# joncampbell123/composite-video-simulator

Hardware: AMD Instinct MI355X
Metric: frames/sec (output frames = fields; 720x486 NTSC, preset '-vhs'; steady-state pipelined throughput, 4 steps in flight) (higher is better)
Workload: dtype f64; 1 GPU; 720x486 30fps 10s colour-bars clip, preset '-vhs': 300 frames -> 600 fields per GPU per step, frame-round-robin over 1 GPU(s); steps_in_flight=4, mode=exact (bit-identical to the reference: fp64, no FMA contraction)

## Files before the change

composite-video-simulator_amd/csrc/ntsc_decode_fast.hip:

```cpp
#include "ntsc_pack.hpp"
#include "ntsc_rowend_plan.hpp"

#pragma clang fp contract(off)

namespace ntscsim {
namespace fastdec {

typedef uint32_t v4u __attribute__((ext_vector_type(4)));
#ifdef NTSC_PLAIN_OUT_STORES
#define NTSC_OUT_STORE(p, v) (*(p) = (v))
#else
#define NTSC_OUT_STORE(p, v) __builtin_nontemporal_store((v), (p))
#endif
typedef __attribute__((address_space(1))) v4u *g_v4u_ptr;
typedef __attribute__((address_space(1))) const v4u *g_cv4u_ptr;
DEV v4u to_v4u(const uint4 &a) { return v4u{a.x, a.y, a.z, a.w}; }
typedef __attribute__((address_space(1))) uint32_t *g_u32_ptr;
typedef __attribute__((address_space(1))) const uint32_t *g_cu32_ptr;

#ifdef NTSC_NO_STEP_SCHED_BARRIER
#define NTSC_STEP_SCHED_BARRIER() ((void)0)
#else
#define NTSC_STEP_SCHED_BARRIER() __builtin_amdgcn_sched_barrier(0)
#endif
// ... 182 lines not shown
        if (pick_next) { e1 = D.w4; e2 = D.w2; o1 = D.w5; o2 = D.w3; }
        else           { e1 = D.w5; e2 = D.w3; o1 = D.w4; o2 = D.w2; }
        y0 = D.y0; y1 = D.y1; y2 = D.y2; y3 = D.y3; y4 = D.y4;
        ieP = D.ieP; qeP = D.qeP; ieN = D.ieN; qeN = D.qeN;
    }
    DEV void to(DemodR &D, bool pick_next) const
    {
        D.c2 = c1; D.c1 = pA - c1; D.c0 = pB - D.c1; D.csum = D.c0 + D.c1 + D.c2;
        D.w0 = 0; D.w1 = 0;
        if (pick_next) { D.w4 = e1; D.w2 = e2; D.w5 = o1; D.w3 = o2; }
        else           { D.w5 = e1; D.w3 = e2; D.w4 = o1; D.w2 = o2; }
        D.y0 = y0; D.y1 = y1; D.y2 = y2; D.y3 = y3; D.y4 = y4;
        D.ieP = ieP; D.qeP = qeP; D.ieN = ieN; D.qeN = qeN;
    }
    template <bool PICK, bool NEG, bool LUMA, bool BK = false, bool MASK = false, bool ANY = false>
    DEV void push(int ct, bool hi, int dm, int &Yo, int &Io, int &Qo, unsigned bmul = 0, unsigned bshift = 0,
                  bool odd = false, int mo = 0)
    {
        const int p = ct + c1;
        const int yb = sdiv4s(p + pB);
        int ch = ct - yb;
        if (BK) ch = scale_back50(ch, bmul, bshift);
        c1 = ct; pB = pA; pA = p;
        if (LUMA) { Yo = y0; y0 = y1; y1 = y2; y2 = y3; y3 = y4; y4 = yb; }
        if (PICK) {
            int a, b;
            if (ANY) {
                const int aL = odd ? o2 : e2, aH = odd ? o1 : e1;
                const int bL = odd ? e1 : o2, bH = odd ? ch : o1;
                a = hi ? aH : aL; b = hi ? bH : bL;
                const int sg = NEG ? ~mo : mo;
                a = (a ^ sg) - sg; b = (b ^ sg) - sg;
            } else {
                a = hi ? e1 : e2; b = hi ? o1 : o2;
                if (NEG) { a = -a; b = -b; }
            }
            e2 = e1; e1 = ch;
            if (MASK) { a &= dm; b &= dm; }
            ieN = a; qeN = b;
            Io = (ieP + ieN) >> 1;
            Qo = (qeP + qeN) >> 1;
        } else {
            o2 = o1; o1 = ch;
            Io = ieN; Qo = qeN;
            ieP = ieN; qeP = qeN;
        }
    }
};

template <bool VHS, class RT>
struct State {
    DemodR D1, D2;
    int l0, l1, l2, lsum;
    Casc3<RT> vl, vcU, vcV, sh, oU, oV;
    PoleHp<RT> vpre;
    int Yprev, Uraw, Vraw;
    RT Uf2[2];
    LaneRand32 rng;
    int nU, nV;
};

template <class RT, bool WR = false, bool BK = false, bool SV = false, bool XA = false, bool FO = false>
struct Const {
    static constexpr bool fullout = FO;
    static constexpr int SH = FO ? 3 : 0;
    RT a_oi, a_oq;
    uint32_t *xs;
    static constexpr bool wraps = WR;
    static constexpr bool back = BK;
    static constexpr bool svideo = SV;
    static constexpr bool anyxi = XA;
    bool odd;
    int mo;
    int ms[4];
    unsigned bmul, bshift;
    int wrapoff;
    int wrapA, wrapS;
    unsigned xi;
    bool hi;
    int W, xe, lane;
    int d, SKT, LOFF;
// ... 48 lines not shown
    g = g < 0 ? 0 : (g > 255 ? 255 : g);
    b = b < 0 ? 0 : (b > 255 ? 255 : b);
    return (((uint32_t)r << 16) | (uint32_t)b) | ((uint32_t)g << 8);
#else
    const uint32_t r = cvt_sat_u32((y + (RT(0.956) * fU)) + (RT(0.621) * fV));
    const uint32_t g = cvt_sat_u32((y + (RT(-0.272) * fU)) + (RT(-0.647) * fV));
    const uint32_t b = cvt_sat_u32((y + (RT(-1.106) * fU)) + (RT(1.703) * fV));
    return pack_bgra(r, g, b);
#endif
}

struct Steady {
    DemodS D1, D2;
    int lc1, lpA, lpB;
    uint32_t *rb;
    bool rb0;
    int yd[4];
    int ud[2];
};

template <int DPH, int J, class RT, class CT>
DEV int vcr_step(const DevParams &P, State<true, RT> &S, Steady &T, const CT &C,
                 int pc, int pl, int &Yv, int &Uv, int &Vv)
{
    constexpr bool pick1 = ((DPH + J) & 1) != 0;
    constexpr bool neg1 = ((DPH + J) & 3) == 3;
    int Yd, U, V;
    T.D1.template push<pick1, neg1, false, CT::back, false, CT::anyxi>(pc, C.hi, -1, Yd, U, V, C.bmul, C.bshift, C.odd, C.mo);
    U += S.nU; V += S.nV;
    S.nU = noise_next(S.nU, S.rng.template draw<2 * J>(T.rb, T.rb0), P.m_cnoise, P.cnoise_k);
    S.nV = noise_next(S.nV, S.rng.template draw<2 * J + 1>(T.rb, T.rb0), P.m_cnoise, P.cnoise_k);
    const RT u = (RT)U, v = (RT)V;
    const RT Ud = rtrunc<RT>((u * C.cosv) - (v * C.sinv));
    const RT Vd = rtrunc<RT>((u * C.sinv) + (v * C.cosv));
    const int fU = (int)S.vcU.push(Ud, C.a_vc);
    const int fV = (int)S.vcV.push(Vd, C.a_vc);
    const int lp = pl + T.lc1;
    const int yb = sdiv4s(lp + T.lpB);
    T.lc1 = pl; T.lpB = T.lpA; T.lpA = lp;
    RT m2;
    RT s = S.vl.push((RT)yb, C.a_vl, m2);
    s += S.vpre.hp(s, m2, C.a_vl) * RT(1.6);
    const RT s0 = rtrunc<RT>(s);
    const RT ts = S.sh.push(s0, C.a_sh);
    const int Y = (int)(s0 + ((s0 - ts) * C.sharp2));
    U = ((wave_up(fU) & C.bA) + fU + C.bC) >> C.bC;
    V = ((wave_up(fV) & C.bA) + fV + C.bC) >> C.bC;
    Yv = Y; Uv = U; Vv = V;
    constexpr int J2 = (J + CT::SH) & 3;
    if constexpr (CT::anyxi) {
        const int chroma = (J2 & 1) ? (C.odd ? U : V) : (C.odd ? V : U);
        const int mm = C.ms[J2];
        return Y + ((chroma ^ mm) - mm);
    }
    const int chroma = (J2 & 1) ? V : U;
    const int mm = (J2 & 2) ? C.mNL : C.mL;
    return Y + ((chroma ^ mm) - mm);
}

template <bool VHS, int DPH, int J, class RT, class CT>
DEV uint32_t step(const DevParams &P, State<VHS, RT> &S, Steady &T, const CT &C, int pc, int pl)
{
    int Y, U, V;
    constexpr bool pick3 = ((J + 1 + CT::SH) & 1) != 0;
    constexpr bool neg3 = ((J + 1 + CT::SH) & 3) == 3;
    if constexpr (!VHS) {
        T.D1.template push<pick3, neg3, true, CT::back, true, CT::anyxi>(pc, C.hi, C.dm, Y, U, V, C.bmul, C.bshift, C.odd, C.mo);
    } else {
        int Yv, Uv, Vv;
        const int c2 = vcr_step<DPH, J, RT, CT>(P, S, T, C, pc, pl, Yv, Uv, Vv);
        if constexpr (CT::svideo) {
            Y = Yv; U = Uv & C.dm; V = Vv & C.dm;
        } else {
            T.D2.template push<pick3, neg3, true, false, true, CT::anyxi>(c2, C.hi, C.dm, Y, U, V, 0, 0, C.odd, C.mo);
        }
    }
    if constexpr (CT::fullout) {
        const int fUn = (int)S.oU.push((RT)U, C.a_oi);
        const RT fVd = rtrunc<RT>(S.oV.push((RT)V, C.a_oq));
        const int Yo = T.yd[J];
        T.yd[J] = Y;
        const RT fUd = (RT)T.ud[J & 1];
        T.ud[J & 1] = fUn;
        return yiq_to_bgra<RT>(Yo, fUd, fVd);
    } else {
// ... 115 lines not shown
    if (in3) {
        fUd = rtrunc<RT>(S.oU.push((RT)U, C.a_tv));
        fVd = rtrunc<RT>(S.oV.push((RT)V, C.a_tv));
    }
    const int xo = x3 - 1;
    const int Yo = S.Yprev;
    const int Ur = S.Uraw, Vr = S.Vraw;
    S.Yprev = Y; S.Uraw = U; S.Vraw = V;
    if (xo < 0) return false;
    if (xo >= W - 1) { fUd = (RT)Ur; fVd = (RT)Vr; }
    px = yiq_to_bgra<RT>(Yo, fUd, fVd);
    xo_out = xo;
    return true;
}

template <bool VHS, int DPH, class RT, class CT>
DEV int steady_run(const DevParams &P, State<VHS, RT> &S, Steady &T, const CT &C, uint32_t *ring,
                   uint32_t *ostage, const unsigned long long *orow, uint32_t *drow, bool is_out, int t, int t_end,
                   int (&pc)[4], int (&pl)[4], int &sbase)
{
    const int SKT = C.SKT, LOFF = C.LOFF, lane = C.lane;
    constexpr int PD = 4;
    constexpr bool PFTOP = !VHS;
    int pend_x = -1;
#ifdef NTSC_FAST_LANE_STORE
#define NTSC_FAST_FLUSH()                                                                         \
    if (pend_x >= 0) {                                                                            \
        if (is_out) {                                                                             \
            const uint4 *sp = reinterpret_cast<const uint4 *>(&ostage[lane * 20]);                \
            g_v4u_ptr dp = (g_v4u_ptr)(drow + pend_x);                                            \
            const uint4 a = sp[0], b = sp[1], c4 = sp[2], d4 = sp[3];                             \
// ... 21 lines not shown
#endif
#ifndef NTSC_FAST_NO_ENTRY_WAIT
    __builtin_amdgcn_s_waitcnt(0x0F70);
#endif
    for (; t + 4 <= t_end; t += 4) {
        if constexpr (FLUSH_TOP) { NTSC_FAST_FLUSH() }
        uint32_t o[4];
        int nc[4] = {0, 0, 0, 0}, nl[4] = {0, 0, 0, 0};
        if (PFTOP) {
#pragma unroll
            for (int j = 0; j < 4; j++) { nc[j] = cs_load(C, t + 4 + j); nl[j] = VHS ? cs_load<NTSC_COMP_LOAD2_AUX>(C, t + 4 + j - LOFF) : 0; }
        }
        T.rb = ring + sbase * 64 + lane;
        T.rb0 = sbase == 0;
        sbase = (sbase + 8) & 31;
#define NTSC_FAST_STEP(J)                                                                         \
        o[J] = step<VHS, DPH, J, RT, CT>(P, S, T, C, pc[J % PD], pl[J % PD]);                     \
        if (!PFTOP) {                                                                             \
            pc[J % PD] = cs_load(C, t + PD + J);                                                  \
            if (VHS) pl[J % PD] = cs_load<NTSC_COMP_LOAD2_AUX>(C, t + PD + J - LOFF);                                  \
        }                                                                                         \
        NTSC_STEP_SCHED_BARRIER();
        NTSC_FAST_STEP(0)
        NTSC_FAST_STEP(1)
        NTSC_FAST_STEP(2)
        NTSC_FAST_STEP(3)
#undef NTSC_FAST_STEP
        if constexpr (PFTOP) {
#pragma unroll
            for (int j = 0; j < 4; j++) { pc[j] = nc[j]; pl[j] = nl[j]; }
        }
        const int xo0 = t - SKT;
        const int sub = (xo0 >> 2) & 3;
        *reinterpret_cast<uint4 *>(&ostage[lane * 20 + sub * 4]) = make_uint4(o[0], o[1], o[2], o[3]);
        if (sub == 3) pend_x = xo0 - 12;
// ... 31 lines not shown
    for (int j = 0; j < PD; j++) { pc[j] = cs_load(C, t + j); pl[j] = VHS ? cs_load<NTSC_COMP_LOAD2_AUX>(C, t + j - LOFF) : 0; }
    t = steady_run<VHS, DPH, RT, CT>(P, S, T, C, ring, ostage, orow, drow, is_out, t, t_end, pc, pl, sbase);
    T.D1.to(S.D1, VHS ? (DPH & 1) != 0 : pick3_next);
    T.D2.to(S.D2, pick3_next);
    if constexpr (CT::fullout) {
#pragma unroll
        for (int q = 0; q < 4; q++) C.xs[q * 64] = (uint32_t)T.yd[q];
        S.Uf2[0] = (RT)T.ud[0]; S.Uf2[1] = (RT)T.ud[1];
    }
    S.Uraw = 0; S.Vraw = 0;
    S.l2 = T.lc1; S.l1 = T.lpA - T.lc1; S.l0 = T.lpB - S.l1; S.lsum = S.l0 + S.l1 + S.l2;
    if (VHS) S.rng.pos = sbase;
    return t;
}

template <int DPH, int J, bool END, class RT, class CT>
DEV uint32_t group_step(const DevParams &P, State<true, RT> &S, Steady &T, const CT &C, const rowend::Pos &q,
                        int t, int pc, int pl)
{
    const int W = C.W;
    constexpr bool pick1 = ((DPH + J) & 1) != 0, neg1 = ((DPH + J) & 3) == 3;
    constexpr bool pick3 = ((J + 1) & 1) != 0, neg3 = ((J + 1) & 3) == 3;
    int Yd, U = 0, V = 0;
    int fU = 0, fV = 0;
    if (!END || q.sep1) {
        if constexpr (END) {
            const int x1 = t - 7;
            const int mg = pick1 ? ((x1 + 2 - W + (C.mL & 2)) >> 31) : -1;
            T.D1.template push<pick1, neg1, false, CT::back, true, false>(pc, C.hi, mg, Yd, U, V, C.bmul, C.bshift);
            if (x1 >= C.xe) { U = 0; V = 0; }
        } else {
            T.D1.template push<pick1, neg1, false, CT::back, false, false>(pc, C.hi, -1, Yd, U, V, C.bmul, C.bshift);
        }
    }
    if (q.in1) {
        U += S.nU; V += S.nV;
        S.nU = noise_next(S.nU, S.rng.template draw<2 * J>(T.rb, T.rb0), P.m_cnoise, P.cnoise_k);
        S.nV = noise_next(S.nV, S.rng.template draw<2 * J + 1>(T.rb, T.rb0), P.m_cnoise, P.cnoise_k);
        const RT u = (RT)U, v = (RT)V;
        const RT Ud = rtrunc<RT>((u * C.cosv) - (v * C.sinv));
        const RT Vd = rtrunc<RT>((u * C.sinv) + (v * C.cosv));
        fU = (int)S.vcU.push(Ud, C.a_vc);
        fV = (int)S.vcV.push(Vd, C.a_vc);
        if (END && q.tail_wr) {
            const int x1 = t - 7;
            C.tailU[(size_t)(x1 & 15) * C.rstride] = (int)Ud;
            C.tailU[(size_t)(16 + (x1 & 15)) * C.rstride] = (int)Vd;
        }
    }
    int yb;
    {
        const int lp = pl + T.lc1;
        yb = sdiv4s(lp + T.lpB);
        T.lc1 = pl; T.lpB = T.lpA; T.lpA = lp;
    }
    int c2 = 0;
    if (q.in2) {
        if (END && q.tail_rd) {
            const int x2 = t - 7 - C.d;
            fU = C.tailU[(size_t)(x2 & 15) * C.rstride];
            fV = C.tailU[(size_t)(16 + (x2 & 15)) * C.rstride];
        }
        RT m2;
        RT s = S.vl.push((RT)yb, C.a_vl, m2);
        s += S.vpre.hp(s, m2, C.a_vl) * RT(1.6);
        const RT s0 = rtrunc<RT>(s);
// ... 18 lines not shown
    }
    uint32_t px = 0;
    if (q.tv) {
        RT fUd = 0, fVd = 0;
        const int Yo = S.Yprev;
        if (q.in3) {
            fUd = rtrunc<RT>(S.oU.push((RT)U3, C.a_tv));
            fVd = rtrunc<RT>(S.oV.push((RT)V3, C.a_tv));
            S.Yprev = Y3;
        }
        if (q.out) px = yiq_to_bgra<RT>(Yo, fUd, fVd);
    }
    return px;
}

template <int DPH, bool END, class RT, class CT>
DEV void group_run(const DevParams &P, State<true, RT> &S, Steady &T, const CT &C, const rowend::Plan &RP,
                   uint32_t *ring, uint32_t *ostage, uint32_t *drow, bool is_out, int t0, int t_stop,
                   int (&pc)[4], int (&pl)[4], int &sbase)
{
    const int lane = C.lane, W = C.W;
    for (; t0 < t_stop; t0 += 4) {
        T.rb = ring + sbase * 64 + lane;
        T.rb0 = sbase == 0;
        sbase = (sbase + 8) & 31;
        uint32_t o[4] = {0u, 0u, 0u, 0u};
        bool burst = false, rest = false;
#define NTSC_GROUP_STEP(J)                                                                        \
        {                                                                                         \
            const int tj = t0 + J;           \
            const rowend::Pos q = rowend::position(RP, tj);                                       \
            o[J] = group_step<DPH, J, END, RT, CT>(P, S, T, C, q, tj, pc[J], pl[J]);              \
            burst = burst || q.burst; rest = rest || q.rest;                                      \
            const int tn = tj + 4;           \
            const rowend::Pos qn = rowend::position(RP, tn);                                      \
            pc[J] = qn.load_c ? cs_load(C, tn) : 0;                                               \
            pl[J] = qn.load_l ? cs_load<NTSC_COMP_LOAD2_AUX>(C, tn - RP.LOFF) : 0;                \
            NTSC_STEP_SCHED_BARRIER();                                                            \
        }
        NTSC_GROUP_STEP(0)
        NTSC_GROUP_STEP(1)
        NTSC_GROUP_STEP(2)
        NTSC_GROUP_STEP(3)
#undef NTSC_GROUP_STEP
        if constexpr (END) {
            const int xo0 = t0 - RP.SKT;
            const int sub = (xo0 >> 2) & 3;
            *reinterpret_cast<uint4 *>(&ostage[lane * 20 + sub * 4]) = make_uint4(o[0], o[1], o[2], o[3]);
            const int xb = xo0 & ~15;
            if (burst) {
                if (is_out) {
                    const uint4 *sp = reinterpret_cast<const uint4 *>(&ostage[lane * 20]);
                    g_v4u_ptr dp = (g_v4u_ptr)(drow + xb);
                    const uint4 a = sp[0], b = sp[1], c4 = sp[2], d4 = sp[3];
                    dp[0] = to_v4u(a); dp[1] = to_v4u(b); dp[2] = to_v4u(c4); dp[3] = to_v4u(d4);
                }
            } else if (rest && is_out) {
                for (int x = xb; x < W; x++) ((g_u32_ptr)drow)[x] = ostage[lane * 20 + (x - xb)];
            }
        }
    }
}


template <int DPH, class RT, class CT>
DEV void grouped_row(const DevParams &P, State<true, RT> &S, const CT &C, const rowend::Plan &RP, uint32_t *ring,
                     uint32_t *ostage, const unsigned long long *orow, uint32_t *drow, bool is_out)
{
    Steady T;
    T.D1.init(); T.D2.init();
    T.lc1 = T.lpA = T.lpB = 0;
    int sbase = rowend::group_slot(S.rng.pos, RP.g0);
    int pc[4], pl[4];
#pragma unroll
    for (int j = 0; j < 4; j++) {
        pc[j] = rowend::position(RP, RP.g0 + j).load_c ? cs_load(C, RP.g0 + j) : 0;
        pl[j] = 0;
    }
    group_run<DPH, false, RT, CT>(P, S, T, C, RP, ring, ostage, drow, is_out, RP.g0, RP.st0, pc, pl, sbase);
    const int t = steady_run<true, DPH, RT, CT>(P, S, T, C, ring, ostage, orow, drow, is_out, RP.st0, RP.t_end, pc, pl, sbase);
#pragma unroll
    for (int j = 0; j < 4; j++) pc[j] = rowend::position(RP, t + j).load_c ? pc[j] : 0;
    group_run<DPH, true, RT, CT>(P, S, T, C, RP, ring, ostage, drow, is_out, t, RP.glast + 4, pc, pl, sbase);
}

}

#ifndef NTSC_FAST_WAVES
#define NTSC_FAST_WAVES 2
#endif
#ifndef NTSC_FAST_WAVES_F32
#define NTSC_FAST_WAVES_F32 2
#endif
template <class RT> struct FastWaves { static constexpr int n = NTSC_FAST_WAVES; };
template <> struct FastWaves<float> { static constexpr int n = NTSC_FAST_WAVES_F32; };
template <bool VHS, class RT, bool WR, bool BK, bool SV = false, bool XA = false, bool FO = false>
DEV void decode_fast_body(const DevParams &P, const GeomDev &G, const FieldDev *__restrict__ fields,
                          const int *__restrict__ comp, const uint32_t *__restrict__ rs_chroma,
                          const int *__restrict__ n0_u, const int *__restrict__ n0_v,
                          const int *__restrict__ hs_shift, const int *__restrict__ pn_noise,
                          const int *__restrict__ dropout, int *__restrict__ tails)
{
    using namespace fastdec;
    __shared__ uint32_t ring[33 * 64];
    __shared__ uint32_t lring[FO ? 12 * 64 : 64];
    __shared__ __attribute__((aligned(16))) uint32_t ostage[64 * 20];
    __shared__ unsigned long long orow[64];

    const int lane = threadIdx.x;
    const int gidx = blockIdx.x * 63 + lane - 1;
    const int rc = gidx < 0 ? 0 : (gidx < P.R ? gidx : P.R - 1);
    const int f = rc / P.Lslot, k = rc - f * P.Lslot;
    const FieldDev &fd = fields[f];
    const unsigned field = fd.field & 1u;
    const bool rowok = (int)(field + 2u * k) < P.H;
#ifdef NTSC_AB_NOSTORE
    const bool is_out = false;
#else
    const bool is_out = lane >= 1 && gidx < P.R && rowok;
#endif
    const unsigned y = rowok ? field + 2u * (unsigned)k : field;
    const int W = P.W;
// ... 46 lines not shown
        C.wrapA = hs > 0 ? tw - hs - 1 : (hs < 0 ? -hs - 1 : 0x3FFFFFFF);
        C.wrapS = opaque_v(hs < 0 ? -1 : 0);
    }
    C.comp = __builtin_amdgcn_make_buffer_rsrc(const_cast<int *>(comp), 0,
                                               (int)((unsigned)W * (unsigned)C.rowbytes), 0x00020000);

    State<VHS, RT> S;
    S.D1.init(); S.D2.init();
    S.l0 = S.l1 = S.l2 = S.lsum = 0;
    S.vl.reset(16, C.a_vl); S.vpre.reset(16, C.a_vl); S.vcU.reset(0, C.a_vc); S.vcV.reset(0, C.a_vc);
    S.sh.reset(0, C.a_sh);
    if (CT::fullout) { S.oU.reset(0, C.a_oi); S.oV.reset(0, C.a_oq); }
    else { S.oU.reset(0, C.a_tv); S.oV.reset(0, C.a_tv); }
    S.Yprev = S.Uraw = S.Vraw = 0;
    C.xs = lring + lane;
    if (CT::fullout)
        for (int q = 0; q < 12; q++) C.xs[q * 64] = 0;
    S.Uf2[0] = S.Uf2[1] = 0;
    S.nU = S.nV = 0;
    if (VHS) {
        S.rng.init(ring, rs_chroma + rc, P.Rpad, lane, rowend::ring_offset(C.SKT));
        S.nU = n0_u[rc]; S.nV = n0_v[rc];
    }

#ifdef NTSC_ROWENDS_OLD
    constexpr bool GROUPS = false;
#else
    constexpr bool GROUPS = VHS && !SV && !XA && !FO;
#endif
    if constexpr (GROUPS) {
        if (rowend::grouped(RP) && (C.d & 3) != 3) {
            switch (C.d & 3) {
                case 0: grouped_row<0, RT, CT>(P, S, C, RP, ring, ostage, orow, drow, is_out); break;
                case 1: grouped_row<1, RT, CT>(P, S, C, RP, ring, ostage, orow, drow, is_out); break;
                default: grouped_row<2, RT, CT>(P, S, C, RP, ring, ostage, orow, drow, is_out); break;
            }
            return;
        }
    }
    const int SKT = C.SKT;
    const int total = W + SKT;
    int t = 0;
#ifdef NTSC_EDGE_UNROLL
#pragma unroll NTSC_EDGE_UNROLL
#endif
    for (; t < SKT && t < total; t++) {
        uint32_t px; int xo;
        (void)edge_step<VHS, RT, CT>(P, S, C, ring, t, px, xo);
    }
// ... 231 lines not shown
```

composite-video-simulator_amd/csrc/ntsc_pack.hpp:

```cpp
#pragma once
#include <stdint.h>

#ifdef __HIPCC__
#define NTSC_PACK_FN __host__ __device__ __forceinline__
#else
#define NTSC_PACK_FN static inline
#endif

namespace ntscsim {

NTSC_PACK_FN uint32_t perm_b32(uint32_t hi, uint32_t lo, uint32_t sel)
{
#ifdef __HIP_DEVICE_COMPILE__
    return __builtin_amdgcn_perm(hi, lo, sel);
#else
    const uint64_t src = ((uint64_t)hi << 32) | lo;
    uint32_t d = 0;
    for (int i = 0; i < 4; i++) {
        const uint32_t s = (sel >> (8 * i)) & 0xFFu;
        const uint32_t byte = s < 8 ? (uint32_t)(src >> (8 * s)) & 0xFFu : 0u;
        d |= byte << (8 * i);
    }
    return d;
#endif
// ... 1 lines not shown

NTSC_PACK_FN uint32_t pack_bgra_shift(uint32_t r, uint32_t g, uint32_t b)
{
    r = r >> 8; g = g >> 8; b = b >> 8;
    r = r < 255u ? r : 255u; g = g < 255u ? g : 255u; b = b < 255u ? b : 255u;
    return ((r << 16) | b) | (g << 8);
}

NTSC_PACK_FN uint32_t pack_bgra_perm(uint32_t r, uint32_t g, uint32_t b)
{
    r = r < 0xFFFFu ? r : 0xFFFFu; g = g < 0xFFFFu ? g : 0xFFFFu; b = b < 0xFFFFu ? b : 0xFFFFu;
    const uint32_t gb = perm_b32(g, b, 0x0c0c0501u);
    return perm_b32(r, gb, 0x0c050100u);
}

NTSC_PACK_FN uint32_t pack_bgra(uint32_t r, uint32_t g, uint32_t b)
{
#ifdef NTSC_PACK_SHIFT
    return pack_bgra_shift(r, g, b);
#else
    return pack_bgra_perm(r, g, b);
#endif
}

}
```

composite-video-simulator_amd/csrc/ntsc_rowend_plan.hpp:

```cpp
#pragma once

#ifdef __HIPCC__
#define NTSC_PLAN_FN __host__ __device__ __forceinline__
#else
#define NTSC_PLAN_FN static inline
#endif

namespace ntscsim {
namespace rowend {

struct Plan {
    int W, d;
    bool vhs, sv, fo;
    int D2;
    int D3;
    int OD;
    int SKT;
    int LOFF;
    int total;
    int t_end;
    int st0, st1;
    int g0;
    int glast;
};
// ... 43 lines not shown
    q.in1 = p.vhs && x1 >= 0 && x1 < W;
    q.in3 = x3 >= 0 && x3 < W;
    q.sep1 = p.vhs ? (t >= 0 && x1 < W) : (t >= 0 && x3 < W);
    q.tail_wr = q.in1 && x1 >= W - p.d;
    q.load_l = p.vhs && xl >= 0 && xl < W;
    q.in2 = p.vhs && x2 >= 0 && x2 < W;
    q.tail_rd = q.in2 && x2 >= W - p.d;
    q.tv = x3 >= 0 && x3 < W + p.OD;
    q.xo = x3 - p.OD;
    q.out = q.tv && q.xo >= 0;
    q.burst = q.out && (q.xo & 15) == 15;
    q.rest = q.out && !q.burst && q.xo == W - 1;
    return q;
}

NTSC_PLAN_FN int ring_offset(int SKT) { return (-(31 + 2 * (SKT - 7))) & 7; }
NTSC_PLAN_FN int group_slot(int first_slot, int t0) { return (first_slot + 2 * (t0 - 7)) & 31; }

}
}
```

composite-video-simulator_amd/csrc/ntscsim_hip.hip:

```cpp
#include <hip/hip_runtime.h>

#include <algorithm>
#include <cmath>
#include <cstdio>
#include <cstdlib>
#include <cstring>
#include <mutex>
#include <new>
#include <string>
#include <vector>

#include "ntscsim.h"
#include "ntsc_device.hpp"
#include "engine_host.hpp"

#include "ntsc_kernels.hip"
#include "ntsc_decode_fast.hip"
#include "ntsc_encode_fast.hip"
#include "ntsc_pipe.hip"
#include "ntsc422_kernels.hip"
#include "ntsc422_fused.hip"
#include "ntsc_scale.hip"
#include "ntsc_float.hpp"
#include "ntsc_stage.hpp"
// ... 91 lines not shown
    std::vector<ScaleDev> host_scale;
    DevBuf<ScaleDev> scale;
    DevBuf<uint32_t> rs_luma, rs_chroma;
    FieldDev *stage[2] = {nullptr, nullptr};
    size_t stage_cap[2] = {0, 0};
    hipEvent_t stage_ev[2] = {nullptr, nullptr};
    bool stage_used[2] = {false, false};
    int stage_idx = 0;
    unsigned char *stage422[2] = {nullptr, nullptr};
    size_t stage422_cap[2] = {0, 0};
    hipEvent_t stage422_ev[2] = {nullptr, nullptr};
    bool stage422_used[2] = {false, false};
    int stage422_idx = 0;

    std::string kernels;
    int last_n = 0, last_W = 0, last_H = 0, last_Rpad = 0, last_Lslot = 0;

    DevBuf<uint8_t> fsrc, fdst;
    struct HostSlot { DevBuf<uint8_t> dsrc, ddst, dyuv, draw; DevBuf<YuvDev> yrec; DevBuf<ScaleDev> srec;
                      hipEvent_t up = nullptr, done = nullptr, down = nullptr; };
    HostSlot hslot[2];
    hipStream_t s_up = nullptr, s_dn = nullptr;
    hipEvent_t ev_src = nullptr;
    bool src_pending = false;
    struct SetupSpec {
        bool have_last = false;
        DevParams D;
        GeomDev G;
        unsigned field = 0, field_before = 0;
        bool armed = false, dry = false;
// ... 381 lines not shown

extern "C" void ntscsim_debug_no_fast_decode(ntscsim_ctx *c, int on)
{
    if (c) { c->no_fast_decode = (on & 1) != 0; c->split_vhs = (on & 2) != 0; c->no_stream422 = (on & 4) != 0; c->no_ghost_fuse = (on & 8) != 0; c->no_setup_merge = (on & 16) != 0; }
}

extern "C" int ntscsim_debug_last_kernels(const ntscsim_ctx *c, char *out, size_t cap)
{
    if (!c || !out || cap == 0) return NTSCSIM_E_ARG;
    std::string kernels = c->kernels;
    if (c->scan) ntscsim::scan_kernels_tap(c->scan, c->device, kernels);
    const size_t n = std::min(cap - 1, kernels.size());
    std::memcpy(out, kernels.data(), n);
    out[n] = 0;
    return (int)kernels.size();
}

extern "C" void ntscsim_debug_set_warmup(ntscsim_ctx *c, int luma_draws, int chroma_draws)
{
    if (!c) return;
    c->warm_override[0] = luma_draws;
    c->warm_override[1] = chroma_draws & ~1;
}

#ifndef NTSC_SETUP_MERGE_MAX
#define NTSC_SETUP_MERGE_MAX 64
#endif
static void launch_setup_kernels(ntscsim_ctx *c, const DevParams &D, const GeomDev &G, const FieldDev *fields_dev, int n, hipStream_t st,
                                 bool note, bool launch)
{
// ... 360 lines not shown
    if (evs) HIPCHK(c, hipEventRecord(evs->e[2], st));
    const bool back50 = D.amp_back == 50;
    const bool dec_base = !c->force_generic && !D.nocolor && D.out_lp == 1 && D.amp == 50;
    const bool dec_common = dec_base && back50;
#define NTSC_LAUNCH_DECODE_RT(VHS, CO, F, RT)                                                   \
    do { note_kernel(c, ("k_decode<" #VHS "," #CO "," + std::to_string((unsigned)(F)) + "u," #RT ">").c_str()); \
    hipLaunchKernelGGL((k_decode<VHS, CO, F, RT>), dgrid, dim3(64), 0, st, D, G, fields_dev,     \
                       dec_in, c->rs_chroma.p, c->n0_u.p, c->n0_v.p, c->hs_shift.p,           \
                       c->pn_noise.p, c->dropout.p, c->tails.p); } while (0)
#define NTSC_LAUNCH_DECODE(VHS, CO, F)                                                          \
    do { if (fast) NTSC_LAUNCH_DECODE_RT(VHS, CO, F, float);                                     \
         else NTSC_LAUNCH_DECODE_RT(VHS, CO, F, double); } while (0)
    const bool dec_fast = dec_base && (back50 || D.amp_back >= 2) && !c->no_fast_decode && D.dst_al16 && even_phase && small_plane;
    const bool dec_fast_xi = dec_base && back50 && !c->no_fast_decode && D.dst_al16 && !even_phase && D.vhs && !D.svideo &&
                             D.cnoise_k && D.pnoise_k && fast_plane_ok((size_t)D.Rpad, W, D.hs ? 2 : 0);
#define NTSC_LAUNCH_FAST(VHS, RT)                                                                \
    do { note_kernel(c, "k_decode_fast<" #VHS "," #RT ">");                                      \
    hipLaunchKernelGGL((k_decode_fast<VHS, RT>), dgrid, dim3(64), 0, st, D, G, fields_dev, dec_in, \
                       c->rs_chroma.p, c->n0_u.p, c->n0_v.p, c->hs_shift.p, c->pn_noise.p,       \
                       c->dropout.p, c->tails.p); } while (0)
#define NTSC_LAUNCH_FAST_BK(VHS, RT)                                                             \
    do { note_kernel(c, "k_decode_fast_bk<" #VHS "," #RT ">");                                   \
    hipLaunchKernelGGL((k_decode_fast_bk<VHS, RT>), dgrid, dim3(64), 0, st, D, G, fields_dev, dec_in, \
                       c->rs_chroma.p, c->n0_u.p, c->n0_v.p, c->hs_shift.p, c->pn_noise.p,       \
                       c->dropout.p, c->tails.p); } while (0)
#define NTSC_LAUNCH_FAST_WR(RT)                                                                  \
    do { note_kernel(c, "k_decode_fast<true," #RT ",true>");                                     \
    hipLaunchKernelGGL((k_decode_fast<true, RT, true>), dgrid, dim3(64), 0, st, D, G, fields_dev, dec_in, \
                       c->rs_chroma.p, c->n0_u.p, c->n0_v.p, c->hs_shift.p, c->pn_noise.p,       \
                       c->dropout.p, c->tails.p); } while (0)
    if (pipe_form || pipe_tv || pipe_tv_catv) {
    } else if (fp) {
        static const int fpv_env = std::getenv("NTSCSIM_FP_VARIANT") ? std::atoi(std::getenv("NTSCSIM_FP_VARIANT")) : -1;
        const int fpv = fpv_env >= 0 ? fpv_env : (n <= 128 ? 0 : 10);
        note_kernel(c, D.vhs ? (fpv < 10 ? "k_decode_fp2" : "k_decode_fp<true>") : "k_decode_fp<false>");
        launch_decode_fp(st, D, G, fields_dev, dec_in, c->rs_chroma.p, c->n0_u.p, c->n0_v.p, c->hs_shift.p, c->pn_noise.p,
                         c->dropout.p, c->tails.p, fpv);
    } else if (dec_fast && back50 && hs_small && D.vhs && !D.svideo && D.cnoise_k && D.pnoise_k && c->split_vhs) {
        HIPCHK(c, c->comp_vcr.ensure((size_t)D.Rpad * W));
        note_kernel(c, fast ? "k_vcr_front<float>" : "k_vcr_front<double>");
        note_kernel(c, fast ? "k_decode_fast<false,float>" : "k_decode_fast<false,double>");
        hipStream_t sv = st, stv = st;
        if (role_probe) {
// ... 1084 lines not shown
```

composite-video-simulator_amd/ntscsim/__init__.py:

```python
import ctypes as C

try:
    import torch
except ImportError:
    pass

from . import _capi
from ._capi import (DESC_BOB, DESC_INTERLACED, DESC_TFF, RNG_AUTO, Field422Desc, FieldDesc,
                    NtscsimError, Out422Desc, YuvDesc, ScaleDesc, HostSource, Params, lib, make_params,
                    make_params_to_composite)

__all__ = ["FieldSimulator", "FrameBlender", "ColorKeyer", "FrameAverager", "Scanimator", "EdgeAligner", "blend_plan", "blend_frame_times", "Pool", "Params", "FieldDesc", "make_params", "NtscsimError", "lib",
           "field_rows", "calls_per_field", "field_schedule"]


def field_rows(height, field):
    return (height - field + 1) // 2 if height > field else 0


def calls_per_field(params, width, height, field):
    return int(lib().ntscsim_rng_calls_per_field(C.byref(params), width, height, field))


def field_schedule(n_fields, first=0):
# ... 292 lines not shown
        return {"setup": out[0], "encode": out[1], "decode": out[2], "total": out[3],
                "calls": n.value}

    def debug_force_generic(self, on=True):
        self._lib.ntscsim_debug_force_generic(self._h, 1 if on else 0)

    def debug_no_fast_decode(self, on=True):
        self._lib.ntscsim_debug_no_fast_decode(self._h, int(on))

    def last_kernels(self):
        buf = C.create_string_buffer(1024)
        n = self._lib.ntscsim_debug_last_kernels(self._h, buf, len(buf))
        if n < 0:
            raise RuntimeError("ntscsim_debug_last_kernels: %d" % n)
        return [k for k in buf.value.decode().split(";") if k]

    def debug_set_warmup(self, luma_draws, chroma_draws):
        self._lib.ntscsim_debug_set_warmup(self._h, int(luma_draws), int(chroma_draws))

    def debug_composite(self, n_fields, width, height):
        import numpy as np
        lslot = (height + 1) // 2
        a = np.zeros((n_fields, lslot, width), dtype=np.int32)
        rc = self._lib.ntscsim_debug_read_composite(
            self._h, a.ctypes.data_as(C.POINTER(C.c_int32)), a.size)
        self._chk(rc, "ntscsim_debug_read_composite")
        return a


def blend_frame_times(params, n_frames, rate_num, rate_den=1):
# ... 533 lines not shown
```

composite-video-simulator_amd/ntscsim/_capi.py:

```python
import ctypes as C
import os

PKG_DIR = os.path.dirname(os.path.dirname(os.path.abspath(__file__)))
PRODUCT_SO = os.environ.get("NTSCSIM_LIB") or os.path.join(PKG_DIR, "libntscsim.so")

OK, E_ARG, E_SIZE, E_NODEV, E_HIP, E_NOMEM, E_PARAM, E_FLAG, E_HELP, E_INTERNAL = \
    0, -1, -2, -3, -4, -5, -6, -7, -8, -9
RNG_AUTO = 0xFFFFFFFFFFFFFFFF
MODE_EXACT, MODE_FAST32, MODE_FLOAT = 0, 1, 2
DESC_INTERLACED, DESC_TFF, DESC_BOB = 1, 2, 0x100
SUBMIT_SAME_SRC, SUBMIT_SRC_STABLE = 0x10000, 0x20000
TICKET_ALL = 0xFFFFFFFFFFFFFFFF

EXPORTS = (
    "ntscsim_params_init", "ntscsim_cli_init", "ntscsim_params_parse_argv",
    "ntscsim_params_validate", "ntscsim_rng_calls_per_field", "ntscsim_rng_draw",
    "ntscsim_create", "ntscsim_destroy", "ntscsim_strerror", "ntscsim_last_error",
    "ntscsim_set_mode", "ntscsim_get_rng_pos", "ntscsim_set_rng_pos", "ntscsim_field", "ntscsim_frames_host",
    "ntscsim_fields_device",
    "ntscsim_batch_create", "ntscsim_batch_run", "ntscsim_batch_destroy",
    "ntscsim_sync", "ntscsim_set_profiling", "ntscsim_get_timings_ms", "ntscsim_set_launch_form",
    "ntscsim_debug_read_composite", "ntscsim_debug_set_warmup",
    "ntscsim_debug_force_generic", "ntscsim_debug_no_fast_decode", "ntscsim_debug_last_kernels", "ntscsim_debug_fast_plane_ok", "ntscsim_debug_field_stats",
    "ntscsim_params_init_to_composite", "ntscsim_params_parse_argv_to_composite",
    "ntscsim_fields422_device", "ntscsim_output422_device", "ntscsim_bgra_to_yuv_device", "ntscsim_rng_calls_per_field_422",
    "ntscsim_scale_to_bgra_device", "ntscsim_frames_host_scaled",
    "ntscsim_batch422_create", "ntscsim_batch422_run", "ntscsim_batch422_destroy",
    "ntscsim_raw28_opts_init", "ntscsim_raw28_parse_argv", "ntscsim_raw28_geometry", "ntscsim_raw28_create",
    "ntscsim_raw28_destroy", "ntscsim_raw28_last_error", "ntscsim_raw28_decode", "ntscsim_raw28_decode_device",
    "ntscsim_raw28_stream_reset", "ntscsim_raw28_stream_push",
    "ntscsim_raw28_get_levels", "ntscsim_raw28_debug_set_speculation", "ntscsim_raw28_debug_stats", "ntscsim_raw28_debug_pick_chunk",
    "ntscsim_raw28_debug_read_front",
    "ntscsim_submit_opts_init", "ntscsim_submit_configure", "ntscsim_submit", "ntscsim_flush", "ntscsim_wait",
    "ntscsim_host_unpin", "ntscsim_submit_stats",
    "ntscsim_host_pin", "ntscsim_host_alloc", "ntscsim_host_free", "ntscsim_host_frame_alloc", "ntscsim_set_pin_policy",
    "ntscsim_field422", "ntscsim_submit422", "ntscsim_submit422_configure", "ntscsim_submit422_stats",
    "ntscsim_pool_create", "ntscsim_pool_destroy", "ntscsim_pool_size", "ntscsim_pool_ctx", "ntscsim_pool_set_block",
    "ntscsim_pool_get_rng_pos", "ntscsim_pool_set_rng_pos", "ntscsim_pool_last_error", "ntscsim_pool_frames_host",
# ... 358 lines not shown
    L.ntscsim_scale_to_bgra_device.argtypes = [C.c_void_p, C.POINTER(ScaleDesc), C.c_int, C.c_int, C.c_int,
                                               C.c_void_p]
    L.ntscsim_scale_to_bgra_device.restype = C.c_int
    L.ntscsim_frames_host_scaled.argtypes = [C.c_void_p, C.POINTER(HostSource), C.POINTER(C.c_uint8), C.c_size_t,
                                             C.c_int, C.POINTER(C.c_uint8), C.c_size_t, C.c_int, C.c_int, C.c_int,
                                             C.c_uint64, C.c_uint32, C.c_int]
    L.ntscsim_frames_host_scaled.restype = C.c_int
    L.ntscsim_rng_calls_per_field_422.argtypes = [C.POINTER(Params), C.c_int, C.c_int, C.c_uint]
    L.ntscsim_rng_calls_per_field_422.restype = C.c_uint64
    L.ntscsim_debug_force_generic.argtypes = [C.c_void_p, C.c_int]
    L.ntscsim_debug_force_generic.restype = None
    L.ntscsim_debug_no_fast_decode.argtypes = [C.c_void_p, C.c_int]
    L.ntscsim_debug_no_fast_decode.restype = None
    L.ntscsim_debug_last_kernels.argtypes = [C.c_void_p, C.c_char_p, C.c_size_t]
    L.ntscsim_debug_last_kernels.restype = C.c_int
    L.ntscsim_debug_fast_plane_ok.argtypes = [C.c_int] * 4
    L.ntscsim_debug_fast_plane_ok.restype = C.c_int
    L.ntscsim_debug_field_stats.argtypes = [C.c_void_p, C.POINTER(C.c_uint64)]
    L.ntscsim_debug_field_stats.restype = None
    L.ntscsim_batch422_create.argtypes = [C.c_void_p, C.POINTER(Field422Desc), C.c_int, C.c_int, C.c_int,
                                          C.POINTER(C.c_void_p)]
    L.ntscsim_batch422_create.restype = C.c_int
    L.ntscsim_batch422_run.argtypes = [C.c_void_p, C.c_void_p]
    L.ntscsim_batch422_run.restype = C.c_int
    L.ntscsim_batch422_destroy.argtypes = [C.c_void_p]
    L.ntscsim_batch422_destroy.restype = None
    L.ntscsim_raw28_opts_init.argtypes = [C.POINTER(Raw28Opts)]
    L.ntscsim_raw28_opts_init.restype = None
    L.ntscsim_raw28_parse_argv.argtypes = [C.POINTER(Raw28Opts), C.c_int, C.POINTER(C.c_char_p), C.c_int]
    L.ntscsim_raw28_parse_argv.restype = C.c_int
# ... 326 lines not shown
```

include/ntscsim.h:

```cpp
#ifndef NTSCSIM_H
#define NTSCSIM_H

#include <stddef.h>
#include <stdint.h>

#ifdef __cplusplus
extern "C" {
#endif

#define NTSCSIM_ABI_VERSION 1

enum {
    NTSCSIM_OK          = 0,
    NTSCSIM_E_ARG       = -1,
    NTSCSIM_E_SIZE      = -2,
    NTSCSIM_E_NODEV     = -3,
    NTSCSIM_E_HIP       = -4,
    NTSCSIM_E_NOMEM     = -5,
    NTSCSIM_E_PARAM     = -6,
    NTSCSIM_E_FLAG      = -7,
    NTSCSIM_E_HELP      = -8,
    NTSCSIM_E_INTERNAL  = -9
};

// ... 288 lines not shown
int ntscsim_set_launch_form(ntscsim_ctx *ctx, int form);

void ntscsim_set_profiling(ntscsim_ctx *ctx, int on);
int  ntscsim_get_timings_ms(ntscsim_ctx *ctx, float out_ms[4], int *n_calls);

int ntscsim_debug_read_composite(ntscsim_ctx *ctx, int32_t *out, size_t out_elems);

void ntscsim_debug_set_warmup(ntscsim_ctx *ctx, int luma_draws, int chroma_draws);

void ntscsim_debug_force_generic(ntscsim_ctx *ctx, int on);

void ntscsim_debug_no_fast_decode(ntscsim_ctx *ctx, int on);

int ntscsim_debug_last_kernels(const ntscsim_ctx *ctx, char *out, size_t cap);

int ntscsim_debug_fast_plane_ok(int n_fields, int width, int height, int head_switching);

void ntscsim_debug_field_stats(const ntscsim_ctx *ctx, uint64_t out[4]);

typedef struct ntscsim_raw28_opts {
    uint32_t struct_size;
    uint32_t _pad0;
    double   sample_rate;
    int32_t  mark_sync;
    int32_t  disable_sync;
    int32_t  disable_wp_equ;
    int32_t  show_subcarrier;
    int32_t  disable_subcarrier;
    int32_t  disable_equalization;
} ntscsim_raw28_opts;
// ... 243 lines not shown
```

Baseline: 827,000 frames/s.

## Reuse demod luma via per-lane LDS ring instead of re-reading composite

In the grouped VHS decode path for delay phase 1 with LOFF 14, the luma box-filter value already computed by the first demodulator is stored in a 16-slot per-lane LDS ring. It is read back 14 samples later instead of issuing a second global composite load and recomputing the sum. This removes one global load stream per sample, at the cost of dynamic LDS per block plus LDS stores and loads. Separately, the default BGRA pack switches to a saturating cvt_pk_u16 plus perm variant.

```diff
diff --git a/composite-video-simulator_amd/csrc/ntsc_decode_fast.hip b/composite-video-simulator_amd/csrc/ntsc_decode_fast.hip
--- a/composite-video-simulator_amd/csrc/ntsc_decode_fast.hip
+++ b/composite-video-simulator_amd/csrc/ntsc_decode_fast.hip
@@ -220,8 +220,8 @@
         D.ieP = ieP; D.qeP = qeP; D.ieN = ieN; D.qeN = qeN;
     }
     template <bool PICK, bool NEG, bool LUMA, bool BK = false, bool MASK = false, bool ANY = false>
-    DEV void push(int ct, bool hi, int dm, int &Yo, int &Io, int &Qo, unsigned bmul = 0, unsigned bshift = 0,
-                  bool odd = false, int mo = 0)
+    DEV int push(int ct, bool hi, int dm, int &Yo, int &Io, int &Qo, unsigned bmul = 0, unsigned bshift = 0,
+                 bool odd = false, int mo = 0)
     {
         const int p = ct + c1;
         const int yb = sdiv4s(p + pB);
@@ -251,6 +251,7 @@
             Io = ieN; Qo = qeN;
             ieP = ieN; qeP = qeN;
         }
+        return yb;
     }
 };
 
@@ -271,6 +272,7 @@
     static constexpr bool fullout = FO;
     static constexpr int SH = FO ? 3 : 0;
     RT a_oi, a_oq;
+    uint32_t *yr;
     uint32_t *xs;
     static constexpr bool wraps = WR;
     static constexpr bool back = BK;
@@ -349,19 +351,28 @@
     DemodS D1, D2;
     int lc1, lpA, lpB;
     uint32_t *rb;
+    uint32_t *yw, *yn;
     bool rb0;
     int yd[4];
     int ud[2];
 };
 
-template <int DPH, int J, class RT, class CT>
+template <int J>
+DEV int luma_take(Steady &T, int yb_now)
+{
+    const int yb = (int)(J < 2 ? T.yw[(J + 2) * 64] : T.yn[(J - 2) * 64]);
+    T.yw[J * 64] = (uint32_t)yb_now;
+    return yb;
+}
+
+template <int DPH, int J, class RT, class CT, bool LR = false>
 DEV int vcr_step(const DevParams &P, State<true, RT> &S, Steady &T, const CT &C,
                  int pc, int pl, int &Yv, int &Uv, int &Vv)
 {
     constexpr bool pick1 = ((DPH + J) & 1) != 0;
     constexpr bool neg1 = ((DPH + J) & 3) == 3;
     int Yd, U, V;
-    T.D1.template push<pick1, neg1, false, CT::back, false, CT::anyxi>(pc, C.hi, -1, Yd, U, V, C.bmul, C.bshift, C.odd, C.mo);
+    const int yb1 = T.D1.template push<pick1, neg1, false, CT::back, false, CT::anyxi>(pc, C.hi, -1, Yd, U, V, C.bmul, C.bshift, C.odd, C.mo);
     U += S.nU; V += S.nV;
     S.nU = noise_next(S.nU, S.rng.template draw<2 * J>(T.rb, T.rb0), P.m_cnoise, P.cnoise_k);
     S.nV = noise_next(S.nV, S.rng.template draw<2 * J + 1>(T.rb, T.rb0), P.m_cnoise, P.cnoise_k);
@@ -370,9 +381,14 @@
     const RT Vd = rtrunc<RT>((u * C.sinv) + (v * C.cosv));
     const int fU = (int)S.vcU.push(Ud, C.a_vc);
     const int fV = (int)S.vcV.push(Vd, C.a_vc);
-    const int lp = pl + T.lc1;
-    const int yb = sdiv4s(lp + T.lpB);
-    T.lc1 = pl; T.lpB = T.lpA; T.lpA = lp;
+    int yb;
+    if constexpr (LR) {
+        yb = luma_take<J>(T, yb1);
+    } else {
+        const int lp = pl + T.lc1;
+        yb = sdiv4s(lp + T.lpB);
+        T.lc1 = pl; T.lpB = T.lpA; T.lpA = lp;
+    }
     RT m2;
     RT s = S.vl.push((RT)yb, C.a_vl, m2);
     s += S.vpre.hp(s, m2, C.a_vl) * RT(1.6);
@@ -393,7 +409,7 @@
     return Y + ((chroma ^ mm) - mm);
 }
 
-template <bool VHS, int DPH, int J, class RT, class CT>
+template <bool VHS, int DPH, int J, class RT, class CT, bool LR = false>
 DEV uint32_t step(const DevParams &P, State<VHS, RT> &S, Steady &T, const CT &C, int pc, int pl)
 {
     int Y, U, V;
@@ -403,7 +419,7 @@
         T.D1.template push<pick3, neg3, true, CT::back, true, CT::anyxi>(pc, C.hi, C.dm, Y, U, V, C.bmul, C.bshift, C.odd, C.mo);
     } else {
         int Yv, Uv, Vv;
-        const int c2 = vcr_step<DPH, J, RT, CT>(P, S, T, C, pc, pl, Yv, Uv, Vv);
+        const int c2 = vcr_step<DPH, J, RT, CT, LR>(P, S, T, C, pc, pl, Yv, Uv, Vv);
         if constexpr (CT::svideo) {
             Y = Yv; U = Uv & C.dm; V = Vv & C.dm;
         } else {
@@ -549,7 +565,7 @@
     return true;
 }
 
-template <bool VHS, int DPH, class RT, class CT>
+template <bool VHS, int DPH, class RT, class CT, bool LR = false>
 DEV int steady_run(const DevParams &P, State<VHS, RT> &S, Steady &T, const CT &C, uint32_t *ring,
                    uint32_t *ostage, const unsigned long long *orow, uint32_t *drow, bool is_out, int t, int t_end,
                    int (&pc)[4], int (&pl)[4], int &sbase)
@@ -601,11 +617,15 @@
         T.rb = ring + sbase * 64 + lane;
         T.rb0 = sbase == 0;
         sbase = (sbase + 8) & 31;
+        if constexpr (LR) {
+            T.yw = C.yr + ((t - SKT) & 15) * 64;
+            T.yn = C.yr + ((t - SKT + 4) & 15) * 64;
+        }
 #define NTSC_FAST_STEP(J)                                                                         \
-        o[J] = step<VHS, DPH, J, RT, CT>(P, S, T, C, pc[J % PD], pl[J % PD]);                     \
+        o[J] = step<VHS, DPH, J, RT, CT, LR>(P, S, T, C, pc[J % PD], pl[J % PD]);                 \
         if (!PFTOP) {                                                                             \
             pc[J % PD] = cs_load(C, t + PD + J);                                                  \
-            if (VHS) pl[J % PD] = cs_load<NTSC_COMP_LOAD2_AUX>(C, t + PD + J - LOFF);                                  \
+            if (VHS && !LR) pl[J % PD] = cs_load<NTSC_COMP_LOAD2_AUX>(C, t + PD + J - LOFF);      \
         }                                                                                         \
         NTSC_STEP_SCHED_BARRIER();
         NTSC_FAST_STEP(0)
@@ -667,7 +687,7 @@
     return t;
 }
 
-template <int DPH, int J, bool END, class RT, class CT>
+template <int DPH, int J, bool END, class RT, class CT, bool LR = false>
 DEV uint32_t group_step(const DevParams &P, State<true, RT> &S, Steady &T, const CT &C, const rowend::Pos &q,
                         int t, int pc, int pl)
 {
@@ -676,14 +696,15 @@
     constexpr bool pick3 = ((J + 1) & 1) != 0, neg3 = ((J + 1) & 3) == 3;
     int Yd, U = 0, V = 0;
     int fU = 0, fV = 0;
+    int yb1 = 0;
     if (!END || q.sep1) {
         if constexpr (END) {
             const int x1 = t - 7;
             const int mg = pick1 ? ((x1 + 2 - W + (C.mL & 2)) >> 31) : -1;
-            T.D1.template push<pick1, neg1, false, CT::back, true, false>(pc, C.hi, mg, Yd, U, V, C.bmul, C.bshift);
+            yb1 = T.D1.template push<pick1, neg1, false, CT::back, true, false>(pc, C.hi, mg, Yd, U, V, C.bmul, C.bshift);
             if (x1 >= C.xe) { U = 0; V = 0; }
         } else {
-            T.D1.template push<pick1, neg1, false, CT::back, false, false>(pc, C.hi, -1, Yd, U, V, C.bmul, C.bshift);
+            yb1 = T.D1.template push<pick1, neg1, false, CT::back, false, false>(pc, C.hi, -1, Yd, U, V, C.bmul, C.bshift);
         }
     }
     if (q.in1) {
@@ -702,7 +723,9 @@
         }
     }
     int yb;
-    {
+    if constexpr (LR) {
+        yb = luma_take<J>(T, yb1);
+    } else {
         const int lp = pl + T.lc1;
         yb = sdiv4s(lp + T.lpB);
         T.lc1 = pl; T.lpB = T.lpA; T.lpA = lp;
@@ -751,7 +774,7 @@
     return px;
 }
 
-template <int DPH, bool END, class RT, class CT>
+template <int DPH, bool END, class RT, class CT, bool LR = false>
 DEV void group_run(const DevParams &P, State<true, RT> &S, Steady &T, const CT &C, const rowend::Plan &RP,
                    uint32_t *ring, uint32_t *ostage, uint32_t *drow, bool is_out, int t0, int t_stop,
                    int (&pc)[4], int (&pl)[4], int &sbase)
@@ -761,18 +784,22 @@
         T.rb = ring + sbase * 64 + lane;
         T.rb0 = sbase == 0;
         sbase = (sbase + 8) & 31;
+        if constexpr (LR) {
+            T.yw = C.yr + ((t0 - RP.SKT) & 15) * 64;
+            T.yn = C.yr + ((t0 - RP.SKT + 4) & 15) * 64;
+        }
         uint32_t o[4] = {0u, 0u, 0u, 0u};
         bool burst = false, rest = false;
 #define NTSC_GROUP_STEP(J)                                                                        \
         {                                                                                         \
             const int tj = t0 + J;           \
             const rowend::Pos q = rowend::position(RP, tj);                                       \
-            o[J] = group_step<DPH, J, END, RT, CT>(P, S, T, C, q, tj, pc[J], pl[J]);              \
+            o[J] = group_step<DPH, J, END, RT, CT, LR>(P, S, T, C, q, tj, pc[J], pl[J]);          \
             burst = burst || q.burst; rest = rest || q.rest;                                      \
             const int tn = tj + 4;           \
             const rowend::Pos qn = rowend::position(RP, tn);                                      \
             pc[J] = qn.load_c ? cs_load(C, tn) : 0;                                               \
-            pl[J] = qn.load_l ? cs_load<NTSC_COMP_LOAD2_AUX>(C, tn - RP.LOFF) : 0;                \
+            pl[J] = (!LR && qn.load_l) ? cs_load<NTSC_COMP_LOAD2_AUX>(C, tn - RP.LOFF) : 0;       \
             NTSC_STEP_SCHED_BARRIER();                                                            \
         }
         NTSC_GROUP_STEP(0)
@@ -800,7 +827,7 @@
 }
 
 
-template <int DPH, class RT, class CT>
+template <int DPH, class RT, class CT, bool LR = false>
 DEV void grouped_row(const DevParams &P, State<true, RT> &S, const CT &C, const rowend::Plan &RP, uint32_t *ring,
                      uint32_t *ostage, const unsigned long long *orow, uint32_t *drow, bool is_out)
 {
@@ -814,11 +841,15 @@
         pc[j] = rowend::position(RP, RP.g0 + j).load_c ? cs_load(C, RP.g0 + j) : 0;
         pl[j] = 0;
     }
-    group_run<DPH, false, RT, CT>(P, S, T, C, RP, ring, ostage, drow, is_out, RP.g0, RP.st0, pc, pl, sbase);
-    const int t = steady_run<true, DPH, RT, CT>(P, S, T, C, ring, ostage, orow, drow, is_out, RP.st0, RP.t_end, pc, pl, sbase);
+    if constexpr (LR) {
+#pragma unroll
+        for (int q = 0; q < rowend::LUMA_RING_SLOTS; q++) C.yr[q * 64] = 0u;
+    }
+    group_run<DPH, false, RT, CT, LR>(P, S, T, C, RP, ring, ostage, drow, is_out, RP.g0, RP.st0, pc, pl, sbase);
+    const int t = steady_run<true, DPH, RT, CT, LR>(P, S, T, C, ring, ostage, orow, drow, is_out, RP.st0, RP.t_end, pc, pl, sbase);
 #pragma unroll
     for (int j = 0; j < 4; j++) pc[j] = rowend::position(RP, t + j).load_c ? pc[j] : 0;
-    group_run<DPH, true, RT, CT>(P, S, T, C, RP, ring, ostage, drow, is_out, t, RP.glast + 4, pc, pl, sbase);
+    group_run<DPH, true, RT, CT, LR>(P, S, T, C, RP, ring, ostage, drow, is_out, t, RP.glast + 4, pc, pl, sbase);
 }
 
 }
@@ -843,6 +874,7 @@
     __shared__ uint32_t lring[FO ? 12 * 64 : 64];
     __shared__ __attribute__((aligned(16))) uint32_t ostage[64 * 20];
     __shared__ unsigned long long orow[64];
+    extern __shared__ uint32_t yring[];
 
     const int lane = threadIdx.x;
     const int gidx = blockIdx.x * 63 + lane - 1;
@@ -919,6 +951,7 @@
     else { S.oU.reset(0, C.a_tv); S.oV.reset(0, C.a_tv); }
     S.Yprev = S.Uraw = S.Vraw = 0;
     C.xs = lring + lane;
+    C.yr = yring + lane;
     if (CT::fullout)
         for (int q = 0; q < 12; q++) C.xs[q * 64] = 0;
     S.Uf2[0] = S.Uf2[1] = 0;
@@ -933,11 +966,16 @@
 #else
     constexpr bool GROUPS = VHS && !SV && !XA && !FO;
 #endif
+#ifdef NTSC_LUMA_REREAD
+    constexpr bool LRING = false;
+#else
+    constexpr bool LRING = true;
+#endif
     if constexpr (GROUPS) {
-        if (rowend::grouped(RP) && (C.d & 3) != 3) {
+        if (rowend::grouped(RP) && (C.d & 3) != 3 && (!LRING || (C.d & 3) != 1 || rowend::luma_ring(RP))) {
             switch (C.d & 3) {
                 case 0: grouped_row<0, RT, CT>(P, S, C, RP, ring, ostage, orow, drow, is_out); break;
-                case 1: grouped_row<1, RT, CT>(P, S, C, RP, ring, ostage, orow, drow, is_out); break;
+                case 1: grouped_row<1, RT, CT, LRING>(P, S, C, RP, ring, ostage, orow, drow, is_out); break;
                 default: grouped_row<2, RT, CT>(P, S, C, RP, ring, ostage, orow, drow, is_out); break;
             }
             return;
diff --git a/composite-video-simulator_amd/csrc/ntsc_pack.hpp b/composite-video-simulator_amd/csrc/ntsc_pack.hpp
--- a/composite-video-simulator_amd/csrc/ntsc_pack.hpp
+++ b/composite-video-simulator_amd/csrc/ntsc_pack.hpp
@@ -39,12 +39,34 @@
     return perm_b32(r, gb, 0x0c050100u);
 }
 
+NTSC_PACK_FN uint32_t cvt_pk_u16(uint32_t a, uint32_t b)
+{
+#ifdef __HIP_DEVICE_COMPILE__
+    typedef unsigned short u16x2 __attribute__((ext_vector_type(2)));
+    union { u16x2 v; uint32_t u; } c;
+    c.v = __builtin_amdgcn_cvt_pk_u16(a, b);
+    return c.u;
+#else
+    a = a < 0xFFFFu ? a : 0xFFFFu; b = b < 0xFFFFu ? b : 0xFFFFu;
+    return a | (b << 16);
+#endif
+}
+
+NTSC_PACK_FN uint32_t pack_bgra_sat(uint32_t r, uint32_t g, uint32_t b)
+{
+    const uint32_t rg = cvt_pk_u16(r, g);
+    b = b < 0xFFFFu ? b : 0xFFFFu;
+    return perm_b32(rg, b, 0x0c050701u);
+}
+
 NTSC_PACK_FN uint32_t pack_bgra(uint32_t r, uint32_t g, uint32_t b)
 {
-#ifdef NTSC_PACK_SHIFT
+#if defined(NTSC_PACK_SHIFT)
     return pack_bgra_shift(r, g, b);
+#elif defined(NTSC_PACK_PERM)
+    return pack_bgra_perm(r, g, b);
 #else
-    return pack_bgra_perm(r, g, b);
+    return pack_bgra_sat(r, g, b);
 #endif
 }
 
diff --git a/composite-video-simulator_amd/csrc/ntsc_rowend_plan.hpp b/composite-video-simulator_amd/csrc/ntsc_rowend_plan.hpp
--- a/composite-video-simulator_amd/csrc/ntsc_rowend_plan.hpp
+++ b/composite-video-simulator_amd/csrc/ntsc_rowend_plan.hpp
@@ -81,6 +81,18 @@
     return q;
 }
 
+constexpr int LUMA_RING_SLOTS = 16;
+constexpr int LUMA_RING_BYTES = LUMA_RING_SLOTS * 64 * 4;
+NTSC_PLAN_FN bool luma_ring(const Plan &p)
+{
+#ifdef NTSC_LUMA_REREAD
+    (void)p;
+    return false;
+#else
+    return p.vhs && !p.sv && !p.fo && p.LOFF == 14 && grouped(p);
+#endif
+}
+
 NTSC_PLAN_FN int ring_offset(int SKT) { return (-(31 + 2 * (SKT - 7))) & 7; }
 NTSC_PLAN_FN int group_slot(int first_slot, int t0) { return (first_slot + 2 * (t0 - 7)) & 31; }
 
diff --git a/composite-video-simulator_amd/csrc/ntscsim_hip.hip b/composite-video-simulator_amd/csrc/ntscsim_hip.hip
--- a/composite-video-simulator_amd/csrc/ntscsim_hip.hip
+++ b/composite-video-simulator_amd/csrc/ntscsim_hip.hip
@@ -129,6 +129,7 @@
     int stage422_idx = 0;
 
     std::string kernels;
+    unsigned dec_lds = 0;
     int last_n = 0, last_W = 0, last_H = 0, last_Rpad = 0, last_Lslot = 0;
 
     DevBuf<uint8_t> fsrc, fdst;
@@ -540,6 +541,11 @@
     std::memcpy(out, kernels.data(), n);
     out[n] = 0;
     return (int)kernels.size();
+}
+
+extern "C" int ntscsim_debug_last_decoder_lds(const ntscsim_ctx *c)
+{
+    return c ? (int)c->dec_lds : NTSCSIM_E_ARG;
 }
 
 extern "C" void ntscsim_debug_set_warmup(ntscsim_ctx *c, int luma_draws, int chroma_draws)
@@ -930,19 +936,21 @@
     const bool dec_fast = dec_base && (back50 || D.amp_back >= 2) && !c->no_fast_decode && D.dst_al16 && even_phase && small_plane;
     const bool dec_fast_xi = dec_base && back50 && !c->no_fast_decode && D.dst_al16 && !even_phase && D.vhs && !D.svideo &&
                              D.cnoise_k && D.pnoise_k && fast_plane_ok((size_t)D.Rpad, W, D.hs ? 2 : 0);
+    c->dec_lds = 0;
+    const unsigned lring_lds = rowend::luma_ring(rowend::make_plan(W, D.cdelay, D.vhs != 0, false, false)) ? (unsigned)rowend::LUMA_RING_BYTES : 0u;
 #define NTSC_LAUNCH_FAST(VHS, RT)                                                                \
-    do { note_kernel(c, "k_decode_fast<" #VHS "," #RT ">");                                      \
-    hipLaunchKernelGGL((k_decode_fast<VHS, RT>), dgrid, dim3(64), 0, st, D, G, fields_dev, dec_in, \
+    do { note_kernel(c, "k_decode_fast<" #VHS "," #RT ">"); c->dec_lds = (VHS) ? lring_lds : 0u;  \
+    hipLaunchKernelGGL((k_decode_fast<VHS, RT>), dgrid, dim3(64), (VHS) ? lring_lds : 0u, st, D, G, fields_dev, dec_in, \
                        c->rs_chroma.p, c->n0_u.p, c->n0_v.p, c->hs_shift.p, c->pn_noise.p,       \
                        c->dropout.p, c->tails.p); } while (0)
 #define NTSC_LAUNCH_FAST_BK(VHS, RT)                                                             \
-    do { note_kernel(c, "k_decode_fast_bk<" #VHS "," #RT ">");                                   \
-    hipLaunchKernelGGL((k_decode_fast_bk<VHS, RT>), dgrid, dim3(64), 0, st, D, G, fields_dev, dec_in, \
+    do { note_kernel(c, "k_decode_fast_bk<" #VHS "," #RT ">"); c->dec_lds = (VHS) ? lring_lds : 0u; \
+    hipLaunchKernelGGL((k_decode_fast_bk<VHS, RT>), dgrid, dim3(64), (VHS) ? lring_lds : 0u, st, D, G, fields_dev, dec_in, \
                        c->rs_chroma.p, c->n0_u.p, c->n0_v.p, c->hs_shift.p, c->pn_noise.p,       \
                        c->dropout.p, c->tails.p); } while (0)
 #define NTSC_LAUNCH_FAST_WR(RT)                                                                  \
-    do { note_kernel(c, "k_decode_fast<true," #RT ",true>");                                     \
-    hipLaunchKernelGGL((k_decode_fast<true, RT, true>), dgrid, dim3(64), 0, st, D, G, fields_dev, dec_in, \
+    do { note_kernel(c, "k_decode_fast<true," #RT ",true>"); c->dec_lds = lring_lds;            \
+    hipLaunchKernelGGL((k_decode_fast<true, RT, true>), dgrid, dim3(64), lring_lds, st, D, G, fields_dev, dec_in, \
                        c->rs_chroma.p, c->n0_u.p, c->n0_v.p, c->hs_shift.p, c->pn_noise.p,       \
                        c->dropout.p, c->tails.p); } while (0)
     if (pipe_form || pipe_tv || pipe_tv_catv) {
diff --git a/composite-video-simulator_amd/ntscsim/__init__.py b/composite-video-simulator_amd/ntscsim/__init__.py
--- a/composite-video-simulator_amd/ntscsim/__init__.py
+++ b/composite-video-simulator_amd/ntscsim/__init__.py
@@ -330,6 +330,12 @@
         if n < 0:
             raise RuntimeError("ntscsim_debug_last_kernels: %d" % n)
         return [k for k in buf.value.decode().split(";") if k]
+
+    def last_decoder_lds(self):
+        n = self._lib.ntscsim_debug_last_decoder_lds(self._h)
+        if n < 0:
+            raise RuntimeError("ntscsim_debug_last_decoder_lds: %d" % n)
+        return n
 
     def debug_set_warmup(self, luma_draws, chroma_draws):
         self._lib.ntscsim_debug_set_warmup(self._h, int(luma_draws), int(chroma_draws))
diff --git a/composite-video-simulator_amd/ntscsim/_capi.py b/composite-video-simulator_amd/ntscsim/_capi.py
--- a/composite-video-simulator_amd/ntscsim/_capi.py
+++ b/composite-video-simulator_amd/ntscsim/_capi.py
@@ -21,7 +21,7 @@
     "ntscsim_batch_create", "ntscsim_batch_run", "ntscsim_batch_destroy",
     "ntscsim_sync", "ntscsim_set_profiling", "ntscsim_get_timings_ms", "ntscsim_set_launch_form",
     "ntscsim_debug_read_composite", "ntscsim_debug_set_warmup",
-    "ntscsim_debug_force_generic", "ntscsim_debug_no_fast_decode", "ntscsim_debug_last_kernels", "ntscsim_debug_fast_plane_ok", "ntscsim_debug_field_stats",
+    "ntscsim_debug_force_generic", "ntscsim_debug_no_fast_decode", "ntscsim_debug_last_kernels", "ntscsim_debug_last_decoder_lds", "ntscsim_debug_fast_plane_ok", "ntscsim_debug_field_stats",
     "ntscsim_params_init_to_composite", "ntscsim_params_parse_argv_to_composite",
     "ntscsim_fields422_device", "ntscsim_output422_device", "ntscsim_bgra_to_yuv_device", "ntscsim_rng_calls_per_field_422",
     "ntscsim_scale_to_bgra_device", "ntscsim_frames_host_scaled",
@@ -410,6 +410,8 @@
     L.ntscsim_debug_no_fast_decode.restype = None
     L.ntscsim_debug_last_kernels.argtypes = [C.c_void_p, C.c_char_p, C.c_size_t]
     L.ntscsim_debug_last_kernels.restype = C.c_int
+    L.ntscsim_debug_last_decoder_lds.argtypes = [C.c_void_p]
+    L.ntscsim_debug_last_decoder_lds.restype = C.c_int
     L.ntscsim_debug_fast_plane_ok.argtypes = [C.c_int] * 4
     L.ntscsim_debug_fast_plane_ok.restype = C.c_int
     L.ntscsim_debug_field_stats.argtypes = [C.c_void_p, C.POINTER(C.c_uint64)]
diff --git a/include/ntscsim.h b/include/ntscsim.h
--- a/include/ntscsim.h
+++ b/include/ntscsim.h
@@ -326,6 +326,8 @@
 
 int ntscsim_debug_last_kernels(const ntscsim_ctx *ctx, char *out, size_t cap);
 
+int ntscsim_debug_last_decoder_lds(const ntscsim_ctx *ctx);
+
 int ntscsim_debug_fast_plane_ok(int n_fields, int width, int height, int head_switching);
 
 void ntscsim_debug_field_stats(const ntscsim_ctx *ctx, uint64_t out[4]);
```

Result: faster. 844,600 frames/s (median of 6 runs) (+2.1%).
